# hwidong-na/PyTorch_Speaker_Verification

Measured on AMD Instinct MI355X. Metric: embeddings/sec + GE2E steps/sec at N=64×M=10, 1/2/4/8 MI355X, higher is better.
Workload: dtype f32; 1 GPU; GE2E train step N=64xM=10 per GPU, T=160, 40 mels, LSTM 3x768, proj 256; preset=c2, global_batch=640, per_gpu_batch=640, seq_len=160, parallelism=dp1 (speaker-sharded GE2E, RCCL grad all-reduce)

## Files before the change

### pytorch_speaker_verification_amd/csrc/sv_bf16.h

```cpp
#pragma once
#include "sv_common.h"
#include "sv_gemm.h"

typedef __bf16 bf16x8_t __attribute__((ext_vector_type(8)));
typedef unsigned short bf16_t;

#define BBK 64

__device__ __forceinline__ f32x16 mfma_bf16(bf16x8_t a, bf16x8_t b, f32x16 c) {
  return __builtin_amdgcn_mfma_f32_32x32x16_bf16(a, b, c, 0, 0, 0);
}

template <int R, int NT, int BK>
struct BTileStage {
  static constexpr int LD = BK + 8;
  static constexpr int C8 = BK / 8;
  static constexpr int NV = (R * C8) / NT;
  static_assert(NV >= 1 && NV * NT == R * C8, "tile/thread mismatch");
  uint4 v[NV];
  template <class Map>
  __device__ __forceinline__ void load(const bf16_t* __restrict__ base, long ld, const Map& map, int k0, int K,
                                       int tid) {
#pragma unroll
    for (int i = 0; i < NV; ++i) {
// ... 89 lines not shown
          sa[j].load(A, lda, mapA, kbeg + (c0 + j) * BBK, kend, tid);
          sb[j].load(B, ldb, mapB, kbeg + (c0 + j) * BBK, kend, tid);
        }
      }
    }
#pragma unroll
    for (int j = 0; j < SC; ++j) {
      if (c0 + j < nk) {
        bf16_t* buf = lds + (DIAG ? 0 : (it & 1) * BUF);
        if (!DIAG || c0 == 0) {
          sa[j].store(buf, tid);
          sb[j].store(buf + BM * LD, tid);
        }
        __syncthreads();
        mfma_ktile_bf<TM, TN, BBK, LD>(buf, buf + BM * LD, wm0, wn0, lane, acc);
        ++it;
      }
    }
  }
  __syncthreads();
}

template <int BM, int BN, int NT, int D, int TM, int TN, class MapA, class MapB>
__device__ __forceinline__ void gemm_mainloop_bf_pipe(const bf16_t* __restrict__ A, long lda, const MapA& mapA,
                                                      const bf16_t* __restrict__ B, long ldb, const MapB& mapB,
                                                      int kbeg, int kend, bf16_t* lds, int tid, int wm0, int wn0,
                                                      f32x16 (&acc)[TM][TN]) {
  using SA = BTileStage<BM, NT, BBK>;
  using SB = BTileStage<BN, NT, BBK>;
  constexpr int LD = BBK + 8;
  constexpr int BUF = (BM + BN) * LD;
  const int lane = tid & 63;
  const int nk = (kend - kbeg + BBK - 1) / BBK;
  SA sa[D];
  SB sb[D];
#pragma unroll
  for (int j = 0; j < D; ++j)
    if (j < nk) {
      sa[j].load(A, lda, mapA, kbeg + j * BBK, kend, tid);
      sb[j].load(B, ldb, mapB, kbeg + j * BBK, kend, tid);
    }
  for (int k0 = 0; k0 < nk; k0 += D) {
#pragma unroll
    for (int j = 0; j < D; ++j) {
      const int kt = k0 + j;
      if (kt < nk) {
        bf16_t* buf = lds + (kt & 1) * BUF;
        sa[j].store(buf, tid);
        sb[j].store(buf + BM * LD, tid);
        if (kt + D < nk) {
          sa[j].load(A, lda, mapA, kbeg + (kt + D) * BBK, kend, tid);
          sb[j].load(B, ldb, mapB, kbeg + (kt + D) * BBK, kend, tid);
        }
        __syncthreads();
        mfma_ktile_bf<TM, TN, BBK, LD>(buf, buf + BM * LD, wm0, wn0, lane, acc);
      }
    }
  }
  __syncthreads();
}

template <int BM, int BN, int NT, int SC, int TM, int TN, class MapA, class MapB>
__device__ __forceinline__ void gemm_mainloop_step(const bf16_t* __restrict__ A, long lda, const MapA& mapA,
                                                   const bf16_t* __restrict__ B, long ldb, const MapB& mapB,
                                                   int kbeg, int kend, bf16_t* lds, int tid, int wm0, int wn0,
                                                   f32x16 (&acc)[TM][TN]) {
  if constexpr (SC > 200)
    gemm_mainloop_bf_rp<BM, BN, NT, SC - 200, TM, TN, MapA, MapB, true>(A, lda, mapA, B, ldb, mapB, kbeg, kend, lds,
                                                                        tid, wm0, wn0, acc);
  else if constexpr (SC > 100)
    gemm_mainloop_bf_pipe<BM, BN, NT, SC - 100, TM, TN>(A, lda, mapA, B, ldb, mapB, kbeg, kend, lds, tid, wm0, wn0,
                                                        acc);
  else
    gemm_mainloop_bf_rp<BM, BN, NT, SC, TM, TN>(A, lda, mapA, B, ldb, mapB, kbeg, kend, lds, tid, wm0, wn0, acc);
}

template <int NS, int NACC, int P>
__device__ __forceinline__ void mfma_lds_pipe(const bf16_t* A0, int mstride, const bf16x8_t (&W)[NS],
                                              f32x16 (&acc)[NACC]) {
  bf16x8_t f[P][NACC];
#pragma unroll
  for (int p = 0; p < P; ++p)
#pragma unroll
    for (int m = 0; m < NACC; ++m) f[p][m] = *reinterpret_cast<const bf16x8_t*>(A0 + m * mstride + 16 * p);
#pragma unroll
  for (int s = 0; s < NS; ++s) {
#pragma unroll
    for (int m = 0; m < NACC; ++m) acc[m] = mfma_bf16(f[s % P][m], W[s], acc[m]);
    if (s + P < NS) {
#pragma unroll
      for (int m = 0; m < NACC; ++m) f[s % P][m] = *reinterpret_cast<const bf16x8_t*>(A0 + m * mstride + 16 * (s + P));
    }
    __builtin_amdgcn_sched_barrier(0);
  }
}

__device__ __forceinline__ bf16_t to_bf(float x) {
  const __bf16 b = (__bf16)x;
  return *reinterpret_cast<const bf16_t*>(&b);
}
__device__ __forceinline__ float from_bf(bf16_t x) { return __uint_as_float((unsigned)x << 16); }
__device__ __forceinline__ float round_bf(float x) { return from_bf(to_bf(x)); }
__device__ __forceinline__ unsigned pack_bf2(float a, float b) {
  typedef __bf16 bf2_t __attribute__((ext_vector_type(2)));
  typedef float fl2_t __attribute__((ext_vector_type(2)));
  return __builtin_bit_cast(unsigned, __builtin_convertvector(fl2_t{a, b}, bf2_t));
}
__device__ __forceinline__ uint2 pack_bf4(float a, float b, float c, float d) {
  return uint2{pack_bf2(a, b), pack_bf2(c, d)};
}
__device__ __forceinline__ float4 unpack_bf4(uint2 p) {
  return float4{__uint_as_float(p.x << 16), __uint_as_float(p.x & 0xffff0000u), __uint_as_float(p.y << 16),
                __uint_as_float(p.y & 0xffff0000u)};
}

__device__ __forceinline__ float bf_sigmoid(float x) { return __builtin_amdgcn_rcpf(1.0f + __expf(-x)); }
__device__ __forceinline__ float bf_tanh(float x) {
  return 2.0f * __builtin_amdgcn_rcpf(1.0f + __expf(-2.0f * x)) - 1.0f;
}

__device__ __forceinline__ float lstm_cell_fwd(const float (&p)[4], const float (&x)[4], float c_prev, float (&a)[4],
                                               float& h) {
#pragma clang fp contract(off)
  a[0] = bf_sigmoid(p[0] + x[0]);
  a[1] = bf_sigmoid(p[1] + x[1]);
  a[2] = bf_tanh(p[2] + x[2]);
  a[3] = bf_sigmoid(p[3] + x[3]);
  const float c = a[1] * c_prev + a[0] * a[2];
  h = a[3] * bf_tanh(c);
  return c;
}

__device__ __forceinline__ float lstm_cell_bwd(float dh, float i, float f, float g, float o, float c, float cp,
                                               float dcf_in, float (&d)[4]) {
#pragma clang fp contract(off)
  const float tc = bf_tanh(c);
  const float dc = dh * o * (1.f - tc * tc) + dcf_in;
  d[0] = dc * g * i * (1.f - i);
  d[1] = dc * cp * f * (1.f - f);
  d[2] = dc * i * (1.f - g * g);
  d[3] = dh * tc * o * (1.f - o);
  return dc * f;
}

#ifndef SV_PDBG
#define SV_PDBG 0
#endif
typedef float f2_t __attribute__((ext_vector_type(2)));
__device__ __forceinline__ f2_t round_bf2(f2_t x) {
  typedef __bf16 bf2_t __attribute__((ext_vector_type(2)));
  const unsigned u = __builtin_bit_cast(unsigned, __builtin_convertvector(x, bf2_t));
  return f2_t{__uint_as_float(u << 16), __uint_as_float(u & 0xffff0000u)};
}
__device__ __forceinline__ f2_t round_bf2(f2_t x, float b) {
  typedef __bf16 bf2_t __attribute__((ext_vector_type(2)));
  const unsigned u = __builtin_bit_cast(unsigned, __builtin_convertvector(x + b, bf2_t));
  return f2_t{__uint_as_float(u << 16), __uint_as_float(u & 0xffff0000u)};
}
__device__ __forceinline__ void pack_dg4(const float (&ddv)[4][4], unsigned (&pr)[4][2], float (&dbs)[4][4]) {
  typedef __bf16 bf2_t __attribute__((ext_vector_type(2)));
#pragma unroll
  for (int q = 0; q < 4; ++q)
#pragma unroll
    for (int p = 0; p < 2; ++p) {
      const unsigned u = __builtin_bit_cast(unsigned, __builtin_convertvector(f2_t{ddv[2 * p][q], ddv[2 * p + 1][q]}, bf2_t));
      pr[q][p] = u;
      const f2_t d = f2_t{dbs[q][2 * p], dbs[q][2 * p + 1]} + f2_t{__uint_as_float(u << 16), __uint_as_float(u & 0xffff0000u)};
      dbs[q][2 * p] = d.x;
      dbs[q][2 * p + 1] = d.y;
    }
}
template <typename V>
__device__ __forceinline__ void add_round_bf16x(V& acc, const V& x, float b) {
#pragma unroll
  for (int i = 0; i < 16; i += 2) {
    const f2_t s = f2_t{acc[i], acc[i + 1]} + round_bf2(f2_t{x[i], x[i + 1]}, b);
    acc[i] = s.x;
    acc[i + 1] = s.y;
  }
}
__device__ __forceinline__ f2_t bf_tanh2(f2_t x) {
#pragma clang fp contract(off)
  const f2_t y = -2.0f * x;
  const f2_t e = f2_t{__expf(y.x), __expf(y.y)};
  const f2_t d = 1.0f + e;
  const f2_t r = f2_t{__builtin_amdgcn_rcpf(d.x), __builtin_amdgcn_rcpf(d.y)};
  return 2.0f * r - 1.0f;
}
__device__ __forceinline__ f2_t bf_sigmoid2(f2_t x) {
#pragma clang fp contract(off)
  const f2_t y = -x;
  const f2_t d = 1.0f + f2_t{__expf(y.x), __expf(y.y)};
  return f2_t{__builtin_amdgcn_rcpf(d.x), __builtin_amdgcn_rcpf(d.y)};
}
__device__ __forceinline__ f2_t lstm_cell_fwd2(const f2_t (&p)[4], const f2_t (&x)[4], f2_t c_prev, f2_t (&a)[4],
                                               f2_t& h) {
#pragma clang fp contract(off)
  a[0] = bf_sigmoid2(p[0] + x[0]);
  a[1] = bf_sigmoid2(p[1] + x[1]);
  a[2] = bf_tanh2(p[2] + x[2]);
  a[3] = bf_sigmoid2(p[3] + x[3]);
  const f2_t c = a[1] * c_prev + a[0] * a[2];
  h = a[3] * bf_tanh2(c);
  return c;
}
__device__ __forceinline__ f2_t lstm_cell_bwd2(f2_t dh, f2_t i, f2_t f, f2_t g, f2_t o, f2_t c, f2_t cp, f2_t dcf_in,
                                               f2_t (&d)[4]) {
#pragma clang fp contract(off)
  const f2_t tc = bf_tanh2(c);
  const f2_t dc = dh * o * (1.f - tc * tc) + dcf_in;
  d[0] = dc * g * i * (1.f - i);
  d[1] = dc * cp * f * (1.f - f);
  d[2] = dc * i * (1.f - g * g);
  d[3] = dh * tc * o * (1.f - o);
  return dc * f;
}
template <class V4, class A4>
__device__ __forceinline__ void lstm_cell_bwd_x4(const V4& dh, const A4& i, const A4& f, const A4& g, const A4& o,
                                                 const V4& c, const V4& cp, float (&dcf)[4], float (&dd)[4][4]) {
#pragma unroll
  for (int p = 0; p < 2; ++p) {
    const int v0 = 2 * p, v1 = 2 * p + 1;
    f2_t d2[4];
    const f2_t r = lstm_cell_bwd2(f2_t{dh[v0], dh[v1]}, f2_t{i[v0], i[v1]}, f2_t{f[v0], f[v1]}, f2_t{g[v0], g[v1]},
                                  f2_t{o[v0], o[v1]}, f2_t{c[v0], c[v1]}, f2_t{cp[v0], cp[v1]},
                                  f2_t{dcf[v0], dcf[v1]}, d2);
    dcf[v0] = r.x;
    dcf[v1] = r.y;
#pragma unroll
    for (int q = 0; q < 4; ++q) {
      dd[v0][q] = d2[q].x;
      dd[v1][q] = d2[q].y;
    }
  }
}

#define BF_BM 64
#define BF_U 32

#define SV_PCNT_ROWS 64
#define SV_PCNT_STRIDE 32
#define SV_SYNC_CHANNELS 8
#define SV_BWD_CH0 4
#define SV_SYNC_CNT 32
#define SV_NSTAMP 8
#define SV_NSTAMP_WG 1024
#define SV_SYNC_STAMP (SV_SYNC_CNT + SV_SYNC_CHANNELS * SV_PCNT_ROWS * SV_PCNT_STRIDE)
#define SV_SYNC_WORDS (SV_SYNC_STAMP + 2 * SV_NSTAMP_WG * SV_NSTAMP)
unsigned* sv_sync_cnt(unsigned* sync, int chan);

extern "C" int sv_persist_fwd_ok(int B, int H);
int sv_persist_fwd_fusex_ok(int H, int F);
int sv_persist_fwd_bf16(int T, int B, int H, const bf16_t* whh_bf, bf16_t* gates, float* c_tm, float* h_tm,
                        bf16_t* h_bf, bf16_t* hT, hipStream_t stream, unsigned* sync, int chan = 0,
                        const bf16_t* x_bf = nullptr, int F = 0, const bf16_t* wih_bf = nullptr,
                        const float* b_ih = nullptr, const float* b_hh = nullptr, hipEvent_t pre = nullptr,
                        hipEvent_t post = nullptr, int counters_zeroed = 0);
extern "C" int sv_persist_bwd_ok(int B, int H);
extern "C" size_t sv_persist_bwd_scratch(int T, int B, int H);
int sv_persist_bm(int B, int H, int cus);
struct DbFin;
int sv_persist_bwd_bf16(int T, int B, int H, const bf16_t* whhT, const bf16_t* acts, const float* c_tm,
                        const float* dhup, int up_full, bf16_t* dg, bf16_t* dgT, bf16_t* dgf, hipStream_t stream,
                        unsigned* sync, float* db_ih = nullptr, float* db_hh = nullptr, hipEvent_t pre = nullptr,
                        hipEvent_t post = nullptr, int chan = 0, int counters_zeroed = 0,
                        DbFin* defer = nullptr);
#define SV_DBF_MAX 3
struct DbFin {
  const float* dbp[SV_DBF_MAX];
  float* db_ih[SV_DBF_MAX];
  float* db_hh[SV_DBF_MAX];
  int n, nrb, G;
};
__host__ __device__ inline int dbfin_blocks(const DbFin& f, int threads) {
  return f.n > 0 ? f.n * ((f.G + threads - 1) / threads) : 0;
}
__device__ __forceinline__ void dbfin_run(const DbFin& f, int blk) {
  const int per = (f.G + (int)blockDim.x - 1) / (int)blockDim.x;
  const int l = blk / per, c = (blk % per) * (int)blockDim.x + (int)threadIdx.x;
  if (l >= f.n || c >= f.G) return;
  const float* p = l == 0 ? f.dbp[0] : l == 1 ? f.dbp[1] : f.dbp[2];
  float* o1 = l == 0 ? f.db_ih[0] : l == 1 ? f.db_ih[1] : f.db_ih[2];
  float* o2 = l == 0 ? f.db_hh[0] : l == 1 ? f.db_hh[1] : f.db_hh[2];
  float s = 0.f;
  for (int r = 0; r < f.nrb; ++r) s += p[(long)r * f.G + c];
  o1[c] = s;
  if (o2) o2[c] = s;
}
int sv_dbfin_launch(const DbFin& f, hipStream_t stream);
int sv_persist3_bwd_launch(dim3 grid, int nub, hipStream_t stream, const bf16_t* whhT, const bf16_t* acts,
                           const float* c_tm, const float* dhup, int up_full, bf16_t* dg, bf16_t* dgT, long lddgT,
                           bf16_t* dgf, int T, int Bp, int B, int H, unsigned* cnt, int xcd, unsigned* sync,
                           unsigned limit, int fault, int dbg, float* dbp);
int sv_persist3_fwd_launch(dim3 grid, int nub, hipStream_t stream, const bf16_t* whh_bf, bf16_t* gates, float* c_tm,
                           float* h_tm, bf16_t* h_bf, bf16_t* hT, long ldhT, int T, int Bp, int B, int H, unsigned* cnt,
                           int xcd, unsigned* status, unsigned limit, int fault, const bf16_t* x_bf = nullptr,
                           int F = 0, const bf16_t* wih_bf = nullptr, const float* b_ih = nullptr,
                           const float* b_hh = nullptr, int dbg = 0);
int sv_persist16_fwd_launch(int nrb, int nub, hipStream_t stream, const bf16_t* whh_bf, bf16_t* gates, float* c_tm,
                            float* h_tm, bf16_t* h_bf, bf16_t* hT, long ldhT, int T, int Bp, int B, int H, unsigned* cnt,
                            int xcd, unsigned* status, unsigned limit, int fault, const bf16_t* x_bf = nullptr,
                            int F = 0, const bf16_t* wih_bf = nullptr, const float* b_ih = nullptr,
                            const float* b_hh = nullptr);
int sv_stream_cus(hipStream_t stream);
int sv_persist_fwd_fits(int B, int H, int cus);
int sv_persist_bwd_fits(int B, int H, int cus);
unsigned sv_persist_limit();
int sv_persist_fault(int bwd);
int sv_wave_fwd_fits(int L, int T, int B, int F, int H, int cus);
int sv_wave_fwd_bf16(int L, int T, int B, int F, int H, const bf16_t* x_bf, const bf16_t* const* w_ih_bf,
                     const bf16_t* const* w_hh_bf, const float* const* b_ih, const float* const* b_hh,
                     bf16_t* const* gates, float* const* c_tm, float* const* h_tm, bf16_t* const* h_bf,
                     bf16_t* const* hT, unsigned* sync, hipStream_t stream, unsigned limit, int fault, hipEvent_t pre,
                     hipEvent_t post, int counters_zeroed = 0);
constexpr int WB_L = 3;
inline long bf16_wiht_ld(int H) { return 4L * H + 64; }

struct WaveBwdArgs {
  const bf16_t* whhT[WB_L];
  const bf16_t* wihT[WB_L];
  const bf16_t* acts[WB_L];
  const float* c[WB_L];
  float* dx[WB_L];
  bf16_t* dgf[WB_L];
  bf16_t* dgT[WB_L];
  float* dbp[WB_L];
  unsigned* cnt[WB_L];
  const float* dh_last;
  unsigned* status;
  unsigned limit;
  long lddgT;
  int T, Bp, B, H, nub, nrb, fault;
  long ldwih;
};
int sv_wave_bwd_launch(const WaveBwdArgs& a, hipStream_t stream);
int sv_wave_bwd_fits(int L, int B, int H, int cus);
size_t sv_wave_bwd_scratch(int L, int T, int B, int H);
int sv_wave_bwd_bf16(int L, int T, int B, int H, const bf16_t* const* whhT, const bf16_t* const* wihT,
                     const bf16_t* const* acts, const float* const* c_tm, const float* dh_last, float* const* dx,
                     bf16_t* const* dgT, void* scratch, unsigned* sync, hipStream_t stream, float* const* db_ih,
                     float* const* db_hh, hipEvent_t pre, hipEvent_t post, long ldwih = 0,
                     int zero_next = 0, int ch0 = 0, int counters_zeroed = 0, DbFin* defer = nullptr);
```

### pytorch_speaker_verification_amd/csrc/sv_bf16.hip

```cpp
#include <vector>
#include <algorithm>
#include "sv_common.h"
#include "sv_gemm.h"
#include "../../include/sv_ge2e.h"
#include "sv_bf16.h"
#include "sv_gemm256.h"
#include "sv_persist_dev.h"


enum { BEPI_STORE = 0, BEPI_SLAB = 1, BEPI_STORE_BF16 = 2 };

template <int BM, int BN, int EPI>
__global__ __launch_bounds__(256) void gemm_bf16_kernel(const bf16_t* __restrict__ A, long lda,
                                                        const bf16_t* __restrict__ B, long ldb, void* __restrict__ Cv,
                                                        long ldc, long slab, int M, int N, int K, int kchunk,
                                                        const float* __restrict__ bias0,
                                                        const float* __restrict__ bias1, float beta) {
  extern __shared__ __attribute__((aligned(16))) bf16_t ldsb[];
  constexpr int TM = BM / 64, TN = BN / 64;
  const int tid = threadIdx.x, lane = tid & 63, w = tid >> 6;
  const int tiles_n = (N + BN - 1) / BN;
  const int nwg = tiles_n * ((M + BM - 1) / BM);
  const int id = xcd_remap(blockIdx.x, nwg);
  const int tn = id % tiles_n, tm = id / tiles_n;
// ... 448 lines not shown
  hipLaunchKernelGGL(lstm_step_fwd_bf16_kernel<3>, grid, dim3(512), BFWD_LDS, s, hp, whh, g, cp, c, h, hb, hT, ldhT,
                     t, Bp, B, H);
}

bool sched_persist(int schedule, int H) {
  return !(schedule & SV_SCHED_PER_STEP) && ((schedule & SV_SCHED_PERSIST) || H == 768);
}
bool sched_wave(int schedule, int H) { return sched_persist(schedule, H) && !(schedule & SV_SCHED_PER_LAYER); }

void launch_bwd_bf16(dim3 grid, hipStream_t s, const bf16_t* dgn, const bf16_t* whhT, const float* up,
                     const float* dcfi, const bf16_t* acts, const float* ct, const float* cp, bf16_t* dg, float* dcfo,
                     bf16_t* dgT, long lddgT, int t, int Bp, int B, int H) {
  hipLaunchKernelGGL(lstm_step_bwd_bf16_kernel<6>, grid, dim3(512), BBWD_LDS, s, dgn, whhT, up, dcfi, acts, ct, cp,
                     dg, dcfo, dgT, lddgT, t, Bp, B, H);
}

struct G8FLayer {
  const bf16_t* A;
  const bf16_t* B;
  const bf16_t* B2;
  float* C1;
  float* C2;
  long lda, ldb, ldb2, ldc1, ldc2;
  int N, n1, tiles;
  int f2;
};
struct G8Full {
  G8FLayer lay[WB_L];
  int K;
  int nsw, S;
  float* part;
  unsigned* flag;
  unsigned* status;
  unsigned limit;
  DbFin fin;
};
__global__ __launch_bounds__(512, 1) void gemm_bf16_8qf_kernel(const G8Full q) {
  extern __shared__ __attribute__((aligned(16))) char smem[];
  const int tid = threadIdx.x, lane = tid & 63, w = tid >> 6;
  const int wr = w >> 2, wc = w & 3;
  const G8FLayer& L2 = q.lay[2];
  const G8FLayer& L1 = q.lay[1];
  const G8FLayer& L0 = q.lay[0];
  const int P = L2.tiles + L1.tiles + L0.tiles;
  if ((int)blockIdx.x >= q.nsw + P) {
    dbfin_run(q.fin, blockIdx.x - q.nsw - P);
    return;
  }
  auto run = [&](int r, int kbeg, int nk, g8_f32x4 (&acc)[8][4], int& l, int& tm, int& tn) {
    l = r < L2.tiles ? 2 : r < L2.tiles + L1.tiles ? 1 : 0;
    const int tile = l == 2 ? r : l == 1 ? r - L2.tiles : r - L2.tiles - L1.tiles;
    const bf16_t* A = l == 2 ? L2.A : l == 1 ? L1.A : L0.A;
    const bf16_t* Bm = l == 2 ? L2.B : l == 1 ? L1.B : L0.B;
    const bf16_t* B2 = l == 2 ? L2.B2 : l == 1 ? L1.B2 : L0.B2;
    const long lda = l == 2 ? L2.lda : l == 1 ? L1.lda : L0.lda;
    const long ldb = l == 2 ? L2.ldb : l == 1 ? L1.ldb : L0.ldb;
    const long ldb2 = l == 2 ? L2.ldb2 : l == 1 ? L1.ldb2 : L0.ldb2;
    const int N = l == 2 ? L2.N : l == 1 ? L1.N : L0.N;
    const int n1 = l == 2 ? L2.n1 : l == 1 ? L1.n1 : L0.n1;
    const int f2 = l == 2 ? L2.f2 : l == 1 ? L1.f2 : L0.f2;
    const int tiles_n = N / G256_BM;
    tn = tile % tiles_n;
    tm = tile / tiles_n;
    g8_tile<0>(A, lda, Bm, ldb, G256AFrag{}, G256Dual{B2, ldb2, n1, f2}, tm, tn, kbeg, nk, smem, acc);
  };
  g8_f32x4 acc[8][4];
  int l, tm, tn;
  if ((int)blockIdx.x < q.nsw) {
    for (int j = blockIdx.x; j < P; j += q.nsw) {
      run(j, 0, q.S, acc, l, tm, tn);
      const __amdgpu_buffer_rsrc_t rp = sv_rsrc(q.part + (long)j * G256_BM * G256_BM, G256_BM * G256_BM * 4u);
#pragma unroll
      for (int i = 0; i < 32; ++i) {
        const g8_f32x4 v = acc[i >> 2][i & 3];
        __builtin_amdgcn_raw_buffer_store_b128(
            u32x4_t{__float_as_uint(v[0]), __float_as_uint(v[1]), __float_as_uint(v[2]), __float_as_uint(v[3])}, rp,
            (unsigned)(i * 512 + tid) * 16u, 0, 16 );
      }
      asm volatile("s_waitcnt vmcnt(0)" ::: "memory");
      __syncthreads();
      if (tid == 0) __hip_atomic_fetch_add(q.flag + j, 1u, __ATOMIC_RELAXED, __HIP_MEMORY_SCOPE_AGENT);
    }
    return;
  }
  const int r = xcd_remap((int)blockIdx.x - q.nsw, P);
  run(r, q.S * G256_BK, q.K / G256_BK - q.S, acc, l, tm, tn);
  if (q.S > 0) {
    if (tid == 0) persist_wait(q.flag + r, 1u, q.status, q.limit, 2u);
    __syncthreads();
    const __amdgpu_buffer_rsrc_t rp = sv_rsrc(q.part + (long)r * G256_BM * G256_BM, G256_BM * G256_BM * 4u);
#pragma unroll
    for (int i = 0; i < 32; ++i) {
      const u32x4_t x = __builtin_amdgcn_raw_buffer_load_b128(rp, (unsigned)(i * 512 + tid) * 16u, 0, 16 );
      acc[i >> 2][i & 3] += g8_f32x4{__uint_as_float(x[0]), __uint_as_float(x[1]), __uint_as_float(x[2]),
                                     __uint_as_float(x[3])};
    }
  }
  float* C1 = l == 2 ? L2.C1 : l == 1 ? L1.C1 : L0.C1;
  float* C2 = l == 2 ? L2.C2 : l == 1 ? L1.C2 : L0.C2;
  const long ldc1 = l == 2 ? L2.ldc1 : l == 1 ? L1.ldc1 : L0.ldc1;
  const long ldc2 = l == 2 ? L2.ldc2 : l == 1 ? L1.ldc2 : L0.ldc2;
  const int n1 = l == 2 ? L2.n1 : l == 1 ? L1.n1 : L0.n1;
  const int f2 = l == 2 ? L2.f2 : l == 1 ? L1.f2 : L0.f2;
  const bool second = tn * G256_BM >= n1;
  g8_epilogue<G8_STORE>(acc, second ? C2 : C1, second ? ldc2 : ldc1, 0, tm, second ? tn - n1 / G256_BM : tn, wr, wc,
                        lane, nullptr, nullptr, 0.f, second && f2 > 0 ? f2 : 1 << 30);
}

}

extern "C" size_t sv_gemm_bf16_workspace(int M, int N, int K);
extern "C" int sv_gemm_bf16(int M, int N, int K, const bf16_t* A, long lda, const bf16_t* B, long ldb, float* C,
                            long ldc, const float* bias0, const float* bias1, float beta, float* workspace,
                            hipStream_t stream);
size_t sv_gemm_bf16_dual_workspace(int M, int N1, int N2, int K) {
  const BPlan p = plan_bf16(M, N1, K);
  size_t fused = p.splitk > 1 ? (size_t)p.splitk * M * (N1 + N2) * sizeof(float) : 0;
  return std::max(fused, std::max(sv_gemm_bf16_workspace(M, N1, K), sv_gemm_bf16_workspace(M, N2, K)));
}
int sv_gemm_bf16_dual(int M, int N1, int N2, int K, const bf16_t* A, long lda, const bf16_t* B1, long ldb1, float* C1,
                      long ldc1, const bf16_t* B2, long ldb2, float* C2, long ldc2, float* workspace,
                      hipStream_t stream) {
  const BPlan p = plan_bf16(M, N1, K);
  const bool fused = p.bm == G256_BM && p.splitk > 1 && gemm256_ok(M, N1 + N2, K) && N1 % G256_BM == 0 &&
                     N2 % G256_BM == 0 && workspace && g8_ok(workspace, N1 + N2, nullptr, nullptr) &&
                     ldb1 % 8 == 0 && ldb2 % 8 == 0 && lda % 8 == 0 && !(((uintptr_t)A | (uintptr_t)B1 | (uintptr_t)B2) & 15);
  if (!fused) {
    int rc = sv_gemm_bf16(M, N1, K, A, lda, B1, ldb1, C1, ldc1, nullptr, nullptr, 0.f, workspace, stream);
    if (rc) return rc;
    return sv_gemm_bf16(M, N2, K, A, lda, B2, ldb2, C2, ldc2, nullptr, nullptr, 0.f, workspace, stream);
  }
  const int N = N1 + N2;
  const int tiles = (M / G256_BM) * (N / G256_BM);
  const long slab = (long)M * N;
  hipLaunchKernelGGL((gemm_bf16_8q_kernel<G8_SLAB, 0>), dim3(tiles, p.splitk), dim3(512), G256_LDS, stream, A, lda, B1,
                     ldb1, (void*)workspace, (long)N, slab, M, N, K, p.kchunk, nullptr, nullptr, 0.f, G256AFrag{},
                     G256Dual{B2, ldb2, N1});
  SV_LAUNCH_CHECK();
  const int grid = (int)std::min<long>((slab + 255) / 256, 4096);
  hipLaunchKernelGGL(slab_reduce_bf_kernel, dim3(grid), dim3(256), 0, stream, workspace, p.splitk, slab, C1, ldc1, M, N,
                     0.f, nullptr, nullptr, nullptr, C2, ldc2, N1);
  SV_LAUNCH_CHECK();
  return SV_OK;
}

constexpr int GNB_BM = 128, GNB_BN = 48, GNB_BK = 64;
__global__ __launch_bounds__(256) void gemm_bf16_narrow_kernel(const bf16_t* __restrict__ A, long lda,
                                                               const bf16_t* __restrict__ B, long ldb,
                                                               float* __restrict__ slab, long slab_stride, int M,
                                                               int N, int K, int kchunk) {
  __shared__ __attribute__((aligned(16))) char lds[2][(GNB_BM + GNB_BN) * 128];
  const int tid = threadIdx.x, lane = tid & 63, w = tid >> 6;
  const int lr = lane & 15, lq = lane >> 4;
  const int m0 = blockIdx.x * GNB_BM, s = blockIdx.y;
  const int kbeg = s * kchunk, nk = (min(K, kbeg + kchunk) - kbeg) / GNB_BK;
  auto fill = [&](int kt, int st) {
    const int k0 = kbeg + kt * GNB_BK;
#pragma unroll
    for (int i = 0; i < 4; ++i) {
      const int q = tid + 256 * i, row = q >> 3, c = (q & 7) ^ (row & 7);
      __builtin_amdgcn_global_load_lds((glb_vptr_t)(A + (long)(m0 + row) * lda + k0 + 8 * c),
                                       (lds_vptr_t)(&lds[st][0] + 16 * (w * 64 + 256 * i)), 16, 0, 0);
    }
#pragma unroll
    for (int i = 0; i < 2; ++i) {
      if (i == 1 && w >= 2) break;
      const int q = tid + 256 * i, row = q >> 3, c = (q & 7) ^ (row & 7);
      const int n = min(row, N - 1);
      __builtin_amdgcn_global_load_lds((glb_vptr_t)(B + (long)n * ldb + k0 + 8 * c),
                                       (lds_vptr_t)(&lds[st][GNB_BM * 128] + 16 * (w * 64 + 256 * i)), 16, 0, 0);
    }
  };
  g8_f32x4 acc[2][3];
#pragma unroll
  for (int i = 0; i < 2; ++i)
#pragma unroll
    for (int j = 0; j < 3; ++j) acc[i][j] = g8_f32x4{0.f, 0.f, 0.f, 0.f};
  if (nk > 0) fill(0, 0);
  for (int kt = 0; kt < nk; ++kt) {
    const int st = kt & 1;
    asm volatile("s_waitcnt vmcnt(0)" ::: "memory");
    __syncthreads();
    if (kt + 1 < nk) fill(kt + 1, st ^ 1);
    const char* As = &lds[st][0];
    const char* Bs = &lds[st][GNB_BM * 128];
#pragma unroll
    for (int ks = 0; ks < GNB_BK / 32; ++ks) {
      const int c = 4 * ks + lq;
      bf16x8_t a[2], b[3];
#pragma unroll
      for (int i = 0; i < 2; ++i) {
        const int row = 32 * w + 16 * i + lr;
        a[i] = *reinterpret_cast<const bf16x8_t*>(As + row * 128 + 16 * (c ^ (row & 7)));
      }
#pragma unroll
      for (int j = 0; j < 3; ++j) {
        const int row = 16 * j + lr;
        b[j] = *reinterpret_cast<const bf16x8_t*>(Bs + row * 128 + 16 * (c ^ (row & 7)));
      }
#pragma unroll
      for (int i = 0; i < 2; ++i)
#pragma unroll
        for (int j = 0; j < 3; ++j) acc[i][j] = mfma16_bf16(b[j], a[i], acc[i][j]);
    }
  }
  float* Cz = slab + (long)s * slab_stride;
#pragma unroll
  for (int i = 0; i < 2; ++i)
#pragma unroll
    for (int j = 0; j < 3; ++j) {
      const int col = 16 * j + 4 * lq;
      if (col < N)
        *reinterpret_cast<g8_f32x4*>(Cz + (long)(m0 + 32 * w + 16 * i + lr) * N + col) = acc[i][j];
    }
}
static bool narrow_bf_ok(int M, int N, int K, long lda, long ldb) {
  return N <= GNB_BN && N % 4 == 0 && M % GNB_BM == 0 && K % GNB_BK == 0 && K >= 4096 &&
         lda % 8 == 0 && ldb % 8 == 0;
}
static int narrow_bf_splitk(int K, int& kchunk) {
  const int sk = std::max(1, std::min(32, K / 1024));
  kchunk = ((K + sk - 1) / sk + GNB_BK - 1) / GNB_BK * GNB_BK;
  return (K + kchunk - 1) / kchunk;
}

extern "C" size_t sv_gemm_bf16_workspace(int M, int N, int K) {
  const BPlan p = plan_bf16(M, N, K);
  size_t nar = 0;
  if (narrow_bf_ok(M, N, K, K, K)) {
    int kchunk;
    nar = (size_t)narrow_bf_splitk(K, kchunk) * M * N * sizeof(float);
  }
  if (p.splitk <= 1) return nar;
  return std::max(nar, (size_t)p.splitk * M * N * sizeof(float));
}

extern "C" int sv_gemm_bf16(int M, int N, int K, const bf16_t* A, long lda, const bf16_t* B, long ldb, float* C,
                            long ldc, const float* bias0, const float* bias1, float beta, float* workspace,
                            hipStream_t stream) {
  if (M <= 0 || N <= 0 || K <= 0 || !A || !B || !C) return SV_EARG;
  if (K % 8 || lda % 8 || ldb % 8 || (((uintptr_t)A | (uintptr_t)B) & 15)) return SV_EALIGN;
  if (workspace && !((uintptr_t)workspace & 15) && narrow_bf_ok(M, N, K, lda, ldb)) {
    int kchunk;
    const int sk = narrow_bf_splitk(K, kchunk);
    const long slab = (long)M * N;
    hipLaunchKernelGGL(gemm_bf16_narrow_kernel, dim3(M / GNB_BM, sk), dim3(256), 0, stream, A, lda, B, ldb, workspace,
                       slab, M, N, K, kchunk);
    SV_LAUNCH_CHECK();
    const int grid = (int)std::min<long>((slab + 255) / 256, 4096);
    hipLaunchKernelGGL(slab_reduce_bf_kernel, dim3(grid), dim3(256), 0, stream, workspace, sk, slab, C, ldc, M, N,
                       beta, bias0, bias1);
    SV_LAUNCH_CHECK();
    return SV_OK;
  }
  const BPlan p = plan_bf16(M, N, K);
  if (p.bm == G256_BM) {
    const int tiles = (M / G256_BM) * (N / G256_BM);
    const long slab = (long)M * N;
    if (p.splitk == 1) {
      launch_g256<G256_STORE, 0>(g8_ok(C, ldc, bias0, bias1), dim3(tiles, 1), stream, A, lda, B, ldb, C, ldc, 0L,
                                 M, N, K, p.kchunk, bias0, bias1, beta);
      SV_LAUNCH_CHECK();
      return SV_OK;
    }
    if (!workspace) return SV_EARG;
    launch_g256<G256_SLAB, 0>(g8_ok(workspace, N, nullptr, nullptr), dim3(tiles, p.splitk), stream, A, lda, B,
                              ldb, workspace, (long)N, slab, M, N, K, p.kchunk, nullptr, nullptr, 0.f);
    SV_LAUNCH_CHECK();
    const int grid = (int)std::min<long>((slab + 255) / 256, 4096);
    hipLaunchKernelGGL(slab_reduce_bf_kernel, dim3(grid), dim3(256), 0, stream, workspace, p.splitk, slab, C, ldc, M, N,
                       beta, bias0, bias1);
    SV_LAUNCH_CHECK();
    return SV_OK;
  }
  if (p.splitk == 1) {
    if (p.bm == 64)
      launch_bf<64, 64, BEPI_STORE>(A, lda, B, ldb, C, ldc, 0, M, N, K, 1, p.kchunk, bias0, bias1, beta, stream);
    else
      launch_bf<128, 128, BEPI_STORE>(A, lda, B, ldb, C, ldc, 0, M, N, K, 1, p.kchunk, bias0, bias1, beta, stream);
    SV_LAUNCH_CHECK();
    return SV_OK;
  }
  if (!workspace) return SV_EARG;
  const long slab = (long)M * N;
  if (p.bm == 64)
    launch_bf<64, 64, BEPI_SLAB>(A, lda, B, ldb, workspace, N, slab, M, N, K, p.splitk, p.kchunk, nullptr, nullptr, 0.f,
                                 stream);
  else
    launch_bf<128, 128, BEPI_SLAB>(A, lda, B, ldb, workspace, N, slab, M, N, K, p.splitk, p.kchunk, nullptr, nullptr,
                                   0.f, stream);
  SV_LAUNCH_CHECK();
  const int grid = (int)std::min<long>((slab + 255) / 256, 4096);
  hipLaunchKernelGGL(slab_reduce_bf_kernel, dim3(grid), dim3(256), 0, stream, workspace, p.splitk, slab, C, ldc, M, N,
                     beta, bias0, bias1);
  SV_LAUNCH_CHECK();
  return SV_OK;
}

extern "C" int sv_gemm_bf16_bf(int M, int N, int K, const bf16_t* A, long lda, const bf16_t* B, long ldb, bf16_t* C,
                               long ldc, const float* bias0, const float* bias1, hipStream_t stream) {
  if (M <= 0 || N <= 0 || K <= 0 || !A || !B || !C) return SV_EARG;
  if (K % 8 || lda % 8 || ldb % 8 || (((uintptr_t)A | (uintptr_t)B) & 15)) return SV_EALIGN;
  const BPlan p = plan_bf16(M, N, K);
  if (p.bm == G256_BM && p.splitk == 1 && g8_ok(nullptr, 0, bias0, bias1) && ldc % 8 == 0 &&
      !((uintptr_t)C & 15) && (size_t)N * 4 <= G8P_BIAS_LDS) {
    const int tiles = (M / G256_BM) * (N / G256_BM);
    const int cus = sv_stream_cus(stream);
    const int grid = std::min(tiles, cus > 0 ? cus : 256);
    const size_t lds = G256_LDS + ((bias0 || bias1) ? (size_t)N * 4 : 0);
    hipLaunchKernelGGL((gemm_bf16_8qp_kernel<G8_STORE_BF16>), dim3(grid), dim3(512), lds, stream, A, lda, B, ldb,
                       (void*)C, ldc, M, N, K, bias0, bias1, 0.f);
  } else if ((long)((M + 127) / 128) * ((N + 127) / 128) < 128) {
    launch_bf<64, 64, BEPI_STORE_BF16>(A, lda, B, ldb, C, ldc, 0, M, N, K, 1, ((K + BBK - 1) / BBK) * BBK, bias0,
                                       bias1, 0.f, stream);
  } else {
    launch_bf<128, 128, BEPI_STORE_BF16>(A, lda, B, ldb, C, ldc, 0, M, N, K, 1, ((K + BBK - 1) / BBK) * BBK, bias0,
                                         bias1, 0.f, stream);
  }
  SV_LAUNCH_CHECK();
  return SV_OK;
}

bool gemm_afrag_ok(int T, int B, int N, int H) {
  return gemm256_ok(T * B, N, 4 * H) && B % 32 == 0 && H % G256_BK == 0 &&
         4 * H / G256_BK < 4096 && (unsigned long long)T * B * B < (1ull << 32);
}
int gemm_bf16_afrag(int T, int B, int H, int N, const bf16_t* dgf, int bm, const bf16_t* Bop, long ldb, float* C,
                    long ldc, float* workspace, hipStream_t stream, const DbFin& fin) {
  const int M = T * B, K = 4 * H;
  const int tiles = (M / G256_BM) * (N / G256_BM);
  const long fs = (long)((B + bm - 1) / bm) * bm * 4 * H;
  const G256AFrag af = g256_afrag(dgf, fs, B, bm, H);
  const BPlan p = plan_bf16(M, N, K);
  if (p.splitk == 1 && g8_ok(C, ldc, nullptr, nullptr)) {
    hipLaunchKernelGGL((gemm_bf16_8q_kernel<G256_STORE, 1>), dim3(tiles + dbfin_blocks(fin, 512)), dim3(512), G256_LDS,
                       stream, nullptr, 0L, Bop, ldb, (void*)C, ldc, 0L, M, N, K, p.kchunk, nullptr, nullptr, 0.f, af,
                       G256Dual{}, fin);
    SV_LAUNCH_CHECK();
    return SV_OK;
  }
  if (int rc = sv_dbfin_launch(fin, stream)) return rc;
  if (p.splitk == 1) {
    launch_g256<G256_STORE, 1>(false, dim3(tiles, 1), stream, nullptr, 0L, Bop, ldb, C, ldc, 0L, M, N, K, p.kchunk,
                               nullptr, nullptr, 0.f, af);
    SV_LAUNCH_CHECK();
    return SV_OK;
  }
  if (!workspace) return SV_EARG;
  const long slab = (long)M * N;
  launch_g256<G256_SLAB, 1>(g8_ok(workspace, N, nullptr, nullptr), dim3(tiles, p.splitk), stream, nullptr, 0L,
                            Bop, ldb, workspace, (long)N, slab, M, N, K, p.kchunk, nullptr, nullptr, 0.f, af);
  SV_LAUNCH_CHECK();
  const int grid = (int)std::min<long>((slab + 255) / 256, 4096);
  hipLaunchKernelGGL(slab_reduce_bf_kernel, dim3(grid), dim3(256), 0, stream, workspace, p.splitk, slab, C, ldc, M, N,
                     0.f, nullptr, nullptr);
  SV_LAUNCH_CHECK();
  return SV_OK;
}

extern "C" int sv_cast_bf16_batch(int n, const float* const* x, bf16_t* const* y, const long* count,
                                  hipStream_t stream);
extern "C" int sv_cast_bf16(const float* x, bf16_t* y, long n, hipStream_t stream) {
  if (!x || !y || n <= 0) return SV_EARG;
  return sv_cast_bf16_batch(1, &x, &y, &n, stream);
}

extern "C" int sv_cast_bf16_batch(int n, const float* const* x, bf16_t* const* y, const long* count,
                                  hipStream_t stream) {
  if (n <= 0 || n > 8 || !x || !y || !count) return SV_EARG;
  CastBatch cb{};
  cb.n = n;
  bool vec = true;
  for (int i = 0; i < n; ++i) {
    if (!x[i] || !y[i] || count[i] <= 0) return SV_EARG;
    cb.x[i] = x[i];
    cb.y[i] = y[i];
    vec = vec && count[i] % 4 == 0 && !((uintptr_t)x[i] & 15) && !((uintptr_t)y[i] & 7);
  }
  for (int i = 0; i < n; ++i) cb.start[i + 1] = cb.start[i] + (vec ? count[i] / 4 : count[i]);
  const int grid = (int)std::min<long>((cb.start[n] + 255) / 256, 8192);
  if (vec)
    hipLaunchKernelGGL(cast_bf16_batch_kernel<true>, dim3(grid), dim3(256), 0, stream, cb);
  else
    hipLaunchKernelGGL(cast_bf16_batch_kernel<false>, dim3(grid), dim3(256), 0, stream, cb);
  SV_LAUNCH_CHECK();
  return SV_OK;
}

int transpose_cast_bf16_batch(int n, const float* const* src, const long* lds, const int* R, const int* C,
                              bf16_t* const* dst, const long* ldd, hipStream_t stream, bf16_t* const* dstr = nullptr,
                              const FramesArgs* frames = nullptr) {
  if (n <= 0 || n > 8) return SV_EARG;
  TCastBatch tb{};
  tb.n = n;
  for (int i = 0; i < n; ++i) {
    if (!src[i] || !(dst[i] || (dstr && dstr[i])) || R[i] <= 0 || C[i] <= 0) return SV_EARG;
    tb.src[i] = src[i];
    tb.dst[i] = dst[i];
    tb.dstr[i] = dstr ? dstr[i] : nullptr;
    tb.lds[i] = lds[i];
    tb.ldd[i] = ldd[i];
    tb.R[i] = R[i];
    tb.C[i] = C[i];
    tb.tx[i] = (C[i] + 63) / 64;
    tb.tile0[i + 1] = tb.tile0[i] + tb.tx[i] * ((R[i] + 63) / 64);
    const bool rv = !tb.dstr[i] || (C[i] % 4 == 0 && !((uintptr_t)tb.dstr[i] & 7));
    if (lds[i] % 4 == 0 && ldd[i] % 8 == 0 && !((uintptr_t)src[i] & 15) && !((uintptr_t)dst[i] & 15) && rv)
      tb.vec |= 1u << i;
  }
  const FramesArgs fa = frames ? *frames : FramesArgs{};
  const int nfr = frames ? fa.nbx * fa.T : 0;
  hipLaunchKernelGGL(transpose_cast_batch_kernel, dim3(nfr + tb.tile0[n]), dim3(256), 0, stream, tb, fa, nfr);
  SV_LAUNCH_CHECK();
  return SV_OK;
}

__global__ __launch_bounds__(256) void frames_to_bf16_kernel(const FramesArgs fa) {
  __shared__ float tile[64][65];
  frames_tile(fa, blockIdx.x, blockIdx.y, tile);
}
static FramesArgs frames_args(const float* x, int B, int T, int F, bf16_t* x_bf, bf16_t* xT, int Bp) {
  return FramesArgs{x, x_bf, xT, B, T, F, Bp, (std::max(B, xT ? Bp : B) + 63) / 64};
}
extern "C" int sv_frames_to_bf16(const float* x, int B, int T, int F, bf16_t* x_bf, bf16_t* xT, int Bp,
                                 hipStream_t stream) {
  if (!x || !x_bf || B <= 0 || T <= 0 || F <= 0 || F > 64 || (xT && Bp < B)) return SV_EARG;
  const FramesArgs fa = frames_args(x, B, T, F, x_bf, xT, Bp);
  hipLaunchKernelGGL(frames_to_bf16_kernel, dim3(fa.nbx, T), dim3(256), 0, stream, fa);
  SV_LAUNCH_CHECK();
  return SV_OK;
}

extern "C" int sv_transpose_cast_bf16(const float* src, long ld_src, int R, int C, bf16_t* dst, long ld_dst,
                                      hipStream_t stream) {
  if (!src || !dst || R <= 0 || C <= 0) return SV_EARG;
  return transpose_cast_bf16_batch(1, &src, &ld_src, &R, &C, &dst, &ld_dst, stream);
}

extern "C" int sv_lstm_layer_fwd_bf16(const bf16_t* x_bf, int T, int B, int F, int H, const bf16_t* w_ih_bf,
                                      const bf16_t* w_hh_bf, const float* b_ih, const float* b_hh, bf16_t* gates,
                                      float* c_tm, float* h_tm, bf16_t* h_bf, bf16_t* hT, hipStream_t stream) {
  if (!x_bf || !w_ih_bf || !w_hh_bf || !gates || !c_tm || !h_tm || !h_bf) return SV_EARG;
  if (T <= 0 || B <= 0 || F <= 0 || H <= 0 || F % 8 || H % 8) return SV_ESHAPE;
  const long BH = (long)B * H, BG = 4L * B * H;
  int rc = sv_gemm_bf16_bf(T * B, 4 * H, F, x_bf, F, w_ih_bf, F, gates, 4L * H, b_ih, b_hh, stream);
  if (rc) return rc;
  hipError_t e = sv_memset0(h_tm, BH * sizeof(float), stream);
  if (e != hipSuccess) return (int)e;
  e = sv_memset0(h_bf, BH * sizeof(bf16_t), stream);
  if (e != hipSuccess) return (int)e;
  const int Bp = (B + 7) & ~7;
  const long ldhT = (long)(T + 1) * Bp;
  if (hT && Bp != B) {
    e = sv_memset0(hT, (size_t)H * ldhT * sizeof(bf16_t), stream);
    if (e != hipSuccess) return (int)e;
  }
  const dim3 grid((H + BF_U - 1) / BF_U, (B + BF_BM - 1) / BF_BM);
  for (int t = 0; t < T; ++t) {
    launch_fwd_bf16(grid, stream, t ? h_bf + t * BH : nullptr, w_hh_bf, gates + t * BG,
                    t ? c_tm + (t - 1) * BH : nullptr, c_tm + t * BH, h_tm + (t + 1) * BH, h_bf + (t + 1) * BH, hT,
                    ldhT, t, Bp, B, H);
    SV_LAUNCH_CHECK();
  }
  return SV_OK;
}

extern "C" size_t sv_lstm_layer_bwd_bf16_workspace(int T, int B, int F, int H) {
  const int TBp = T * ((B + 7) & ~7);
  size_t g = sv_gemm_bf16_workspace(4 * H, H, TBp);
  g = std::max(g, sv_gemm_bf16_workspace(4 * H, F, TBp));
  g = std::max(g, sv_gemm_bf16_workspace(T * B, F, 4 * H));
  return 2 * ((size_t)B * H * sizeof(float) + 256) + g + 256;
}

extern "C" int sv_lstm_layer_bwd_bf16(int T, int B, int F, int H, const bf16_t* xT_bf, long ld_xT,
                                      const bf16_t* wihT_bf, const bf16_t* whhT_bf, const bf16_t* gates,
                                      const float* c_tm, const bf16_t* hT_bf, const float* dh_up, int dh_up_full,
                                      bf16_t* dg_bf, bf16_t* dgT_bf, float* dx_tm, float* dw_ih, float* dw_hh,
                                      float* db_ih, float* db_hh, float* workspace, hipStream_t stream) {
  if (!xT_bf || !wihT_bf || !whhT_bf || !gates || !c_tm || !hT_bf || !dg_bf || !dgT_bf || !dw_ih || !dw_hh || !db_ih ||
      !workspace)
    return SV_EARG;
  if (T <= 0 || B <= 0 || F <= 0 || H <= 0 || F % 8 || H % 8 || ld_xT % 8) return SV_ESHAPE;
  const long BH = (long)B * H, BG = 4L * B * H;
  const int Bp = (B + 7) & ~7;
  const int TBp = T * Bp;
  const size_t dcfsz = ((size_t)BH * sizeof(float) + 255) / 256 * 256 / sizeof(float);
  float* dcf0 = workspace;
  float* dcf1 = workspace + dcfsz;
  float* gws = workspace + 2 * dcfsz;
  if (Bp != B) {
    hipError_t e = sv_memset0(dgT_bf, (size_t)4 * H * TBp * sizeof(bf16_t), stream);
    if (e != hipSuccess) return (int)e;
  }
  const dim3 grid((H + BF_U - 1) / BF_U, (B + BF_BM - 1) / BF_BM);
  for (int t = T - 1; t >= 0; --t) {
    const float* up = nullptr;
    if (dh_up) up = dh_up_full ? dh_up + t * BH : (t == T - 1 ? dh_up : nullptr);
    float* dcf_out = (t & 1) ? dcf1 : dcf0;
    const float* dcf_in = (t == T - 1) ? nullptr : ((t & 1) ? dcf0 : dcf1);
    launch_bwd_bf16(grid, stream, t == T - 1 ? nullptr : dg_bf + (t + 1) * BG, whhT_bf, up, dcf_in, gates + t * BG,
                    c_tm + t * BH, t ? c_tm + (t - 1) * BH : nullptr, dg_bf + t * BG, dcf_out, dgT_bf, (long)TBp, t,
                    Bp, B, H);
    SV_LAUNCH_CHECK();
  }
  const long ldhT = (long)(T + 1) * Bp;
  int rc = sv_gemm_bf16(4 * H, H, TBp, dgT_bf, TBp, hT_bf, ldhT, dw_hh, H, nullptr, nullptr, 0.f, gws, stream);
  if (rc) return rc;
  rc = sv_gemm_bf16(4 * H, F, TBp, dgT_bf, TBp, xT_bf, ld_xT, dw_ih, F, nullptr, nullptr, 0.f, gws, stream);
  if (rc) return rc;
  hipLaunchKernelGGL(rowsum_bf16_kernel, dim3(4 * H), dim3(256), 0, stream, dgT_bf, (long)TBp, TBp, db_ih, db_hh);
  SV_LAUNCH_CHECK();
  if (dx_tm) {
    rc = sv_gemm_bf16(T * B, F, 4 * H, dg_bf, 4L * H, wihT_bf, 4L * H, dx_tm, F, nullptr, nullptr, 0.f, gws, stream);
    if (rc) return rc;
  }
  return SV_OK;
}

extern "C" int sv_lstm_stack_fwd_bf16(int L, int T, int B, int F, int H, const bf16_t* x_bf,
                                      const bf16_t* const* w_ih_bf, const bf16_t* const* w_hh_bf,
                                      const float* const* b_ih, const float* const* b_hh, bf16_t* const* gates,
                                      float* const* c_tm, float* const* h_tm, bf16_t* const* h_bf,
                                      bf16_t* const* hT, int chunk, hipStream_t main, const hipStream_t* side,
                                      hipEvent_t* ev, void* sync_block, hipEvent_t* probe, int schedule) {
  if (L <= 0 || !x_bf || !w_ih_bf || !w_hh_bf || !gates || !c_tm || !h_tm || !h_bf || !side || !ev || chunk <= 0)
    return SV_EARG;
  if (schedule & ~SV_SCHED_MASK) return SV_EARG;
  unsigned* sync = reinterpret_cast<unsigned*>(sync_block);
  if (T <= 0 || B <= 0 || F <= 0 || H <= 0 || F % 8 || H % 8) return SV_ESHAPE;
  const int nch = (T + chunk - 1) / chunk;
  const long BH = (long)B * H, BG = 4L * B * H;
  const int Bp = (B + 7) & ~7;
  const long ldhT = (long)(T + 1) * Bp;
  hipError_t e;
  auto zero_state = [&](int l, hipStream_t s) -> int {
    if ((e = sv_memset0(h_tm[l], BH * sizeof(float), s)) != hipSuccess) return (int)e;
    if ((e = sv_memset0(h_bf[l], BH * sizeof(bf16_t), s)) != hipSuccess) return (int)e;
    if (hT[l] && Bp != B && (e = sv_memset0(hT[l], (size_t)H * ldhT * sizeof(bf16_t), s)) != hipSuccess)
      return (int)e;
    return SV_OK;
  };
  auto zero_states = [&](hipStream_t s, bool cnt) -> int {
    void* p[SV_ZB_MAX];
    size_t b[SV_ZB_MAX];
    int n = 0;
    for (int l = 0; l < L; ++l) {
      if (n + 3 > SV_ZB_MAX) {
        if (int rc = sv_zero_bytes_multi(n, p, b, s)) return rc;
        n = 0;
      }
      p[n] = h_tm[l], b[n++] = BH * sizeof(float);
      p[n] = h_bf[l], b[n++] = BH * sizeof(bf16_t);
      if (hT[l] && Bp != B) p[n] = hT[l], b[n++] = (size_t)H * ldhT * sizeof(bf16_t);
    }
    if (cnt) {
      if (n == SV_ZB_MAX) {
        if (int rc = sv_zero_bytes_multi(n, p, b, s)) return rc;
        n = 0;
      }
      p[n] = sync + SV_SYNC_CNT, b[n++] = (size_t)SV_SYNC_CHANNELS * SV_PCNT_ROWS * SV_PCNT_STRIDE * sizeof(unsigned);
    }
    return sv_zero_bytes_multi(n, p, b, s);
  };
  int rc;
  if (sched_wave(schedule, H) && sv_wave_fwd_fits(L, T, B, F, H, sv_stream_cus(main))) {
    if (!sync || L > SV_SYNC_CHANNELS) return SV_EARG;
    if ((rc = zero_states(main, true))) return rc;
    return sv_wave_fwd_bf16(L, T, B, F, H, x_bf, w_ih_bf, w_hh_bf, b_ih, b_hh, gates, c_tm, h_tm, h_bf, hT, sync, main,
                            sv_persist_limit(), sv_persist_fault(0), probe ? probe[0] : nullptr,
                            probe ? probe[1] : nullptr, 1);
  }
  if (sched_persist(schedule, H) && sv_persist_fwd_fits(B, H, sv_stream_cus(main))) {
    if (!sync) return SV_EARG;
    const bool own = L <= SV_BWD_CH0;
    if ((rc = zero_states(main, true))) return rc;
    for (int l = 0; l < L; ++l) {
      const int Fl = l == 0 ? F : H;
      const bf16_t* in = l == 0 ? x_bf : h_bf[l - 1] + BH;
      if (l == 0 && sv_persist_fwd_fusex_ok(H, F)) {
        if ((rc = sv_persist_fwd_bf16(T, B, H, w_hh_bf[l], gates[l], c_tm[l], h_tm[l], h_bf[l], hT[l], main, sync,
                                      own ? l : 0, x_bf, F, w_ih_bf[l], b_ih[l], b_hh[l],
                                      probe ? probe[2 * l] : nullptr, probe ? probe[2 * l + 1] : nullptr, own)))
          return rc;
        continue;
      }
      rc = sv_gemm_bf16_bf(T * B, 4 * H, Fl, in, Fl, w_ih_bf[l], Fl, gates[l], 4L * H, b_ih[l], b_hh[l], main);
      if (rc) return rc;
      if ((rc = sv_persist_fwd_bf16(T, B, H, w_hh_bf[l], gates[l], c_tm[l], h_tm[l], h_bf[l], hT[l], main, sync,
                                    own ? l : 0, nullptr, 0, nullptr, nullptr, nullptr,
                                    probe ? probe[2 * l] : nullptr, probe ? probe[2 * l + 1] : nullptr, own)))
        return rc;
    }
    return SV_OK;
  }
  if (sync && (rc = sv_zero_bytes(sync + SV_SYNC_CNT + (size_t)SV_BWD_CH0 * SV_PCNT_ROWS * SV_PCNT_STRIDE,
                                  (size_t)(SV_SYNC_CHANNELS - SV_BWD_CH0) * SV_PCNT_ROWS * SV_PCNT_STRIDE *
                                      sizeof(unsigned),
                                  main)))
    return rc;
  hipEvent_t ev_start = ev[L * nch];
  e = hipEventRecord(ev_start, main);
  if (e != hipSuccess) return (int)e;
  for (int l = 0; l < L; ++l) {
    hipStream_t s = side[l];
    if ((e = hipStreamWaitEvent(s, ev_start, 0)) != hipSuccess) return (int)e;
// ... 425 lines not shown
```

Before: 11220 embeddings/s.

## Add weight-stationary persistent GEMM for K=768 bf16 projections

Adds a persistent kernel for bf16 GEMMs with K=768. Each workgroup keeps a 256-column slice of B in registers and LDS, then streams 32-row blocks of A through it. Loading the A block, storing the previous C block and adding bias are interleaved with the MFMA loop, so weights are loaded once per CU instead of once per tile. This targets the layer-2/3 LSTM input projections (K=768). It risks heavy register pressure at one wave per SIMD, and with short M and few blocks per CU it may not beat the tiled path.

```diff
diff --git a/pytorch_speaker_verification_amd/csrc/sv_bf16.h b/pytorch_speaker_verification_amd/csrc/sv_bf16.h
--- a/pytorch_speaker_verification_amd/csrc/sv_bf16.h
+++ b/pytorch_speaker_verification_amd/csrc/sv_bf16.h
@@ -415,6 +415,9 @@
                             int xcd, unsigned* status, unsigned limit, int fault, const bf16_t* x_bf = nullptr,
                             int F = 0, const bf16_t* wih_bf = nullptr, const float* b_ih = nullptr,
                             const float* b_hh = nullptr);
+int sv_k1ws_ok(int N, int K, long lda, long ldb, long ldc, int cus);
+int sv_k1ws_launch(int M, int N, const bf16_t* A, const bf16_t* B, bf16_t* C, long ldc, const float* bias0,
+                   const float* bias1, int cus, hipStream_t stream);
 int sv_stream_cus(hipStream_t stream);
 int sv_persist_fwd_fits(int B, int H, int cus);
 int sv_persist_bwd_fits(int B, int H, int cus);
diff --git a/pytorch_speaker_verification_amd/csrc/sv_bf16.hip b/pytorch_speaker_verification_amd/csrc/sv_bf16.hip
--- a/pytorch_speaker_verification_amd/csrc/sv_bf16.hip
+++ b/pytorch_speaker_verification_amd/csrc/sv_bf16.hip
@@ -774,6 +774,11 @@
   if (M <= 0 || N <= 0 || K <= 0 || !A || !B || !C) return SV_EARG;
   if (K % 8 || lda % 8 || ldb % 8 || (((uintptr_t)A | (uintptr_t)B) & 15)) return SV_EALIGN;
   const BPlan p = plan_bf16(M, N, K);
+  const int cus_ws = K == 768 ? sv_stream_cus(stream) : 0;
+  if (sv_k1ws_ok(N, K, lda, ldb, ldc, cus_ws > 0 ? cus_ws : 256) && ldc % 8 == 0 && !((uintptr_t)C & 15)) {
+    if (M > (1 << 30)) return SV_EARG;
+    return sv_k1ws_launch(M, N, A, B, C, ldc, bias0, bias1, cus_ws > 0 ? cus_ws : 256, stream);
+  }
   if (p.bm == G256_BM && p.splitk == 1 && g8_ok(nullptr, 0, bias0, bias1) && ldc % 8 == 0 &&
       !((uintptr_t)C & 15) && (size_t)N * 4 <= G8P_BIAS_LDS) {
     const int tiles = (M / G256_BM) * (N / G256_BM);
diff --git a/pytorch_speaker_verification_amd/csrc/sv_k1ws.hip b/pytorch_speaker_verification_amd/csrc/sv_k1ws.hip
--- /dev/null
+++ b/pytorch_speaker_verification_amd/csrc/sv_k1ws.hip
@@ -0,0 +1,152 @@
+#include "sv_persist_dev.h"
+#include "../../include/sv_ge2e.h"
+
+template <int NL>
+struct K1wsLds {
+  static constexpr int BM = 32, K = 768, LDA = K + 8, CW = 128 + 16;
+  static constexpr int as = 0, cst = as + 2 * BM * LDA * 2, bsum = cst + 4 * BM * CW, wl = bsum + 256 * 4;
+  static constexpr int bytes = wl + wstat_wl_bytes(NL);
+  static_assert(bytes <= SV_LDS_BYTES, "LDS of a CU");
+};
+template <int NL, int PA>
+__global__ __launch_bounds__(256, 1) void gemm_bf16_ws768_kernel(const bf16_t* __restrict__ A,
+                                                                const bf16_t* __restrict__ B, bf16_t* __restrict__ C,
+                                                                long ldc, int M, int nub, int R,
+                                                                const float* __restrict__ bias0,
+                                                                const float* __restrict__ bias1) {
+  using Lds = K1wsLds<NL>;
+  constexpr int NS = 48, K = Lds::K, BM = Lds::BM, LDA = Lds::LDA, CW = Lds::CW, NR = NS - NL;
+  constexpr int ABUF = BM * LDA;
+  extern __shared__ __attribute__((aligned(16))) char smem[];
+  bf16_t* As = reinterpret_cast<bf16_t*>(smem + Lds::as);
+  float* bsum = reinterpret_cast<float*>(smem + Lds::bsum);
+  char* wl = smem + Lds::wl;
+  const int tid = threadIdx.x, lane = tid & 63, g = tid >> 6;
+  const int r = lane & 31, hh = lane >> 5;
+  char* cst = smem + Lds::cst + g * BM * CW;
+  int ub, rg;
+  persist_tile(1, nub, ub, rg);
+  ub = __builtin_amdgcn_readfirstlane(ub);
+  rg = __builtin_amdgcn_readfirstlane(rg);
+  const int n0 = ub * 256;
+  const int nrb = (M + BM - 1) / BM;
+  const int nb = (nrb - rg + R - 1) / R;
+  bf16x8_t wa[NS], wb[NR];
+  {
+    const bf16_t* ra = B + (long)(n0 + 64 * g + r) * K + 8 * hh;
+    wstat_load_split<NS, NL>(ra, ra + 32L * K, true, true, wl, g, lane, wa, wb);
+  }
+  auto wl_read = [&](int j) { return wstat_wl_read<NL>(wl, g, lane, j); };
+  {
+    float x = 0.f;
+    if (bias0) x += bias0[n0 + tid];
+    if (bias1) x += bias1[n0 + tid];
+    bsum[tid] = x;
+  }
+  constexpr int CH = 12;
+  const int srow = tid >> 4, sc = tid & 15;
+  auto stage_load = [&](int blk, uint4 (&v)[CH]) {
+    const int left = M - blk * BM;
+    const int valid = __builtin_amdgcn_readfirstlane(left < 0 ? 0 : (left > BM ? BM : left));
+    const __amdgpu_buffer_rsrc_t ra = sv_rsrc(A + (long)blk * BM * K, (unsigned)(valid * K * 2));
+#pragma unroll
+    for (int i = 0; i < CH; ++i) {
+      const int row = 16 * (i / 6) + srow, c = sc + 16 * (i % 6);
+      const u32x4_t x = __builtin_amdgcn_raw_buffer_load_b128(ra, (unsigned)(row * K * 2 + c * 16), 0, 0);
+      v[i] = uint4{x.x, x.y, x.z, x.w};
+    }
+  };
+  auto stage_store = [&](bf16_t* buf, const uint4 (&v)[CH], int i) {
+    const int row = 16 * (i / 6) + srow, c = sc + 16 * (i % 6);
+    *reinterpret_cast<uint4*>(buf + row * LDA + c * 8) = v[i];
+  };
+  struct CDesc {
+    __amdgpu_buffer_rsrc_t rc;
+    int valid;
+  };
+  auto c_desc = [&](int blk) {
+    const int left = blk < 0 ? 0 : M - blk * BM;
+    CDesc d;
+    d.valid = __builtin_amdgcn_readfirstlane(left > BM ? BM : left);
+    d.rc = sv_rsrc(C + (long)(blk < 0 ? 0 : blk) * BM * ldc + n0,
+                   d.valid > 0 ? (unsigned)((((long)d.valid - 1) * ldc + 256) * 2) : 0u);
+    return d;
+  };
+  auto c_read = [&](int j) { return *reinterpret_cast<const uint4*>(cst + (8 * j + (lane >> 3)) * CW + (lane & 7) * 16); };
+  auto c_store = [&](const CDesc& d, int j, uint4 x) {
+    const int row = 8 * j + (lane >> 3), c = lane & 7;
+    const unsigned off = row < d.valid ? (unsigned)(((long)row * ldc + 64 * g + 8 * c) * 2) : 0xFFFFFFF0u;
+    __builtin_amdgcn_raw_buffer_store_b128(u32x4_t{x.x, x.y, x.z, x.w}, d.rc, off, 0, 2 );
+  };
+  uint4 v[CH];
+  stage_load(rg, v);
+#pragma unroll
+  for (int j = 0; j < CH; ++j) stage_store(As, v, j);
+  for (int i = 0; i < nb; ++i) {
+    const int blk = rg + i * R;
+    asm volatile("s_waitcnt lgkmcnt(0)" ::: "memory");
+    __builtin_amdgcn_s_barrier();
+    __builtin_amdgcn_sched_barrier(0);
+    stage_load(blk + R, v);
+    const CDesc dp = c_desc(i > 0 ? blk - R : -1);
+    bf16_t* nxt = As + ((i + 1) & 1) * ABUF;
+    float4 bq[8];
+    __builtin_amdgcn_sched_barrier(0);
+    f32x16 acc0, acc1;
+#pragma unroll
+    for (int e = 0; e < 16; ++e) acc0[e] = acc1[e] = 0.f;
+    {
+      const bf16_t* A0 = As + (i & 1) * ABUF + r * LDA + 8 * hh;
+      auto afrag = [&](int s) { return *reinterpret_cast<const bf16x8_t*>(A0 + 16 * s); };
+      bf16x8_t fa[PA], wq[2];
+      uint4 cx;
+#pragma unroll
+      for (int p = 0; p < PA; ++p) fa[p] = afrag(p);
+#pragma unroll
+      for (int s = 0; s < NS; ++s) {
+        acc0 = mfma_bf16(wa[s], fa[s % PA], acc0);
+        acc1 = mfma_bf16(s < NR ? wb[s < NR ? s : 0] : wq[s & 1], fa[s % PA], acc1);
+        if (s + PA < NS) fa[s % PA] = afrag(s + PA);
+        if (s + 2 >= NR && s + 2 < NS) wq[s & 1] = wl_read(s + 2 - NR);
+        if (s < 24 && s % 6 == 2) cx = c_read(s / 6);
+        if (s < 24 && s % 6 == 4) c_store(dp, s / 6, cx);
+        if (s >= 28 && s < 28 + CH) stage_store(nxt, v, s - 28);
+        if (s == 42) {
+#pragma unroll
+          for (int hq = 0; hq < 8; ++hq)
+            bq[hq] = *reinterpret_cast<const float4*>(bsum + 64 * g + 32 * (hq >> 2) + 8 * (hq & 3) + 4 * hh);
+        }
+        __builtin_amdgcn_sched_barrier(0);
+      }
+    }
+#pragma unroll
+    for (int h = 0; h < 2; ++h)
+#pragma unroll
+      for (int q = 0; q < 4; ++q) {
+        const int col = 32 * h + 8 * q + 4 * hh;
+        const float4 b4 = bq[4 * h + q];
+        const f32x16& a = h ? acc1 : acc0;
+        *reinterpret_cast<uint2*>(cst + r * CW + col * 2) =
+            pack_bf4(a[4 * q] + b4.x, a[4 * q + 1] + b4.y, a[4 * q + 2] + b4.z, a[4 * q + 3] + b4.w);
+      }
+  }
+  {
+    const CDesc dl = c_desc(rg + (nb - 1) * R);
+#pragma unroll
+    for (int j = 0; j < 4; ++j) c_store(dl, j, c_read(j));
+  }
+}
+
+int sv_k1ws_ok(int N, int K, long lda, long ldb, long ldc, int cus) {
+  return K == 768 && lda == 768 && ldb == 768 && N % 256 == 0 && N / 256 <= cus && ldc >= N && ldc < (1L << 24);
+}
+
+int sv_k1ws_launch(int M, int N, const bf16_t* A, const bf16_t* B, bf16_t* C, long ldc, const float* bias0,
+                   const float* bias1, int cus, hipStream_t stream) {
+  constexpr int NL = 10;
+  const int nub = N / 256, nrb = (M + 31) / 32;
+  const int R = std::min(cus / nub, nrb);
+  hipLaunchKernelGGL((gemm_bf16_ws768_kernel<NL, 4>), dim3(nub * R), dim3(256), K1wsLds<NL>::bytes, stream, A, B, C, ldc,
+                     M, nub, R, bias0, bias1);
+  return (int)hipGetLastError();
+}
```

After: 11190 embeddings/s. No clear change (-0.3%).
